# mmorise/World

Hardware: NVIDIA H100
Metric: analysis frames/sec (Harvest+CheapTrick+D4C) (higher is better)
Workload: dtype f64

## Files before the change

### world_b200/csrc/wb_f0common.cu

```cuda
#include "wb_internal.h"
#include "wb_f0common.cuh"
#include "wb_mma.cuh"
#include <stdlib.h>

namespace wb {

WB_KERNEL(256, 3) fir_plain_kernel(FirParams p) {
  WB_DYN_SMEM(double, smem);
  const int tid = WB_TID, nth = WB_NTH;
  const int T = 2048, R = 8, G = T / R;
  const int u = blockIdx.y, n0 = blockIdx.x * T;
  const int qlen = p.base_len[u] + p.extra_len;
  if (n0 >= qlen) return;
  const int ntaps = p.ntaps;
  const int seg_len = T + ntaps - 1;
  const int seg_cap = seg_len + 16;
  double *seg = smem;
  double *hrev = seg + (seg_cap + (seg_cap >> 3) + 8);
  const double *in = p.in + (size_t)u * p.in_stride + p.in_origin;
  double *out = p.out + (size_t)u * p.out_stride + p.out_origin;
  for (int j = tid; j < ntaps + 8; j += nth) hrev[j] = j < ntaps ? __ldg(&p.taps_rev[j]) : 0.0;
  const int m0 = n0 - ntaps + 1;
  for (int i = tid; i < seg_len + 8; i += nth) seg[pad8(i)] = (i < seg_len) ? in[m0 + i] : 0.0;
  WB_SYNC();
// ... 18 lines not shown
}

#ifndef WB_RING
#define WB_RING 256
#endif
#define WB_FCHUNK 256
struct Trains {
  const double *g[4];
  double *xr, *yr;
  int cap;
  int ifrom[4];
  double afs;
};
WB_DEV double edge_at(const Trains &T, int q, int i) {
  int s = i;
  while (s >= T.cap) s -= T.cap;
  return T.g[q][s];
}
WB_DEV double loc_at(const Trains &T, int q, int j) {
  return j >= T.ifrom[q] ? T.xr[q * WB_RING + (j & (WB_RING - 1))] : (edge_at(T, q, j) + edge_at(T, q, j + 1)) / 2.0 / T.afs;
}
WB_DEV double val_at(const Trains &T, int q, int j) {
  return j >= T.ifrom[q] ? T.yr[q * WB_RING + (j & (WB_RING - 1))] : T.afs / (edge_at(T, q, j + 1) - edge_at(T, q, j));
}

WB_DEV double train_value(const Trains &T, int q, int count, int n_int, double t) {
  const int k = imin(n_int - 1, imax(1, count));
  const double x0 = loc_at(T, q, k - 1), x1 = loc_at(T, q, k);
  const double y0 = val_at(T, q, k - 1), y1 = val_at(T, q, k);
  const double s = (t - x0) / (x1 - x0);
  return y0 + s * (y1 - y0);
}

WB_DEV int first_frame_at_or_after(double x, double frame_period) {
  int g = (int)ceil(x * 1000.0 / frame_period);
  if (g < 0) g = 0;
  while (g > 0 && !((g - 1) * frame_period / 1000.0 < x)) --g;
  while (g * frame_period / 1000.0 < x) ++g;
  return g;
}

#ifdef WB_EMU
static inline void smem_add_u64(unsigned long long *p, unsigned long long v) { *p += v; }
#else
__device__ __forceinline__ void smem_add_u64(unsigned long long *p, unsigned long long v) { atomicAdd(p, v); }
#endif

WB_DEV unsigned long long scan_packed(unsigned long long *c, int G, unsigned long long carry,
                                      unsigned long long *warp_tot ) {
#ifdef WB_EMU
  (void)warp_tot;
  unsigned long long run = carry;
  for (int g = 0; g < G; ++g) { const unsigned long long v = c[g]; c[g] = run; run += v; }
  return run;
#else
  const int tid = threadIdx.x, lane = tid & 31, w = tid >> 5, nw = G >> 5;
  const unsigned long long v = c[tid];
  unsigned long long inc = v;
  for (int o = 1; o < 32; o <<= 1) {
    const unsigned long long t = __shfl_up_sync(0xffffffffu, inc, o);
    if (lane >= o) inc += t;
  }
  if (lane == 31) warp_tot[w] = inc;
  __syncthreads();
  unsigned long long base = carry, all = carry;
  for (int i = 0; i < nw; ++i) { const unsigned long long t = warp_tot[i]; if (i < w) base += t; all += t; }
  c[tid] = base + inc - v;
  __syncthreads();
  return all;
#endif
}

WB_DEV void sweep_store_candidate(const SweepParams &p, int grp, double v0, double v1, double v2, double v3, int i,
                                  double bf, double *cand, double *score) {
  double c = (v0 + v1 + v2 + v3) / 4.0, sc = 0.0;
  const double f0_floor = grp < 0 ? p.f0_floor : p.grp_floor[grp], f0_ceil = grp < 0 ? p.f0_ceil : p.grp_ceil[grp];
  if (p.mode == 0) {
    sc = sqrt(((v0 - c) * (v0 - c) + (v1 - c) * (v1 - c) + (v2 - c) * (v2 - c) + (v3 - c) * (v3 - c)) / 3.0);
    if (c > bf || c < bf / 2.0 || c > f0_ceil || c < f0_floor) { c = 0.0; sc = 100000.0; }
  } else {
    if (c > bf * 1.1 || c < bf * 0.9 || c > f0_ceil || c < f0_floor) c = 0.0;
  }
  cand[i] = c;
  if (score) score[i] = sc / (c + kTiny);
}

WB_DEV void finalize_frames(const SweepParams &p, int grp, const Trains &T, int *lo_j, const int *ni, int f_begin, int f_end,
                            unsigned long long *marks, unsigned long long *orig, unsigned long long *scan_tmp,
                            double bf, double *cand, double *score) {
  const int tid = WB_TID, nth = WB_NTH;
  for (int c0 = f_begin; c0 < f_end; c0 += WB_FCHUNK) {
    const int c1 = imin(f_end, c0 + WB_FCHUNK);
    for (int i = tid; i < WB_FCHUNK; i += nth) marks[i] = 0ull;
    WB_SYNC();
    for (int q = 0; q < 4; ++q)
      for (int j = lo_j[q] + tid; j < ni[q]; j += nth) {
        int m = first_frame_at_or_after(loc_at(T, q, j), p.frame_period);
        if (m < c0) m = c0;
        if (m < c1) smem_add_u64(&marks[m - c0], 1ull << (16 * q));
      }
    WB_SYNC();
    for (int i = tid; i < WB_FCHUNK; i += nth) orig[i] = marks[i];
    WB_SYNC();
    const unsigned long long all = scan_packed(marks, WB_FCHUNK, 0ull, scan_tmp);
    for (int i = tid; i < c1 - c0; i += nth) {
      const unsigned long long inc = marks[i] + orig[i];
      const double t = (c0 + i) * p.frame_period / 1000.0;
      const double v0 = train_value(T, 0, lo_j[0] + (int)(inc & 0xffffull), ni[0], t);
      const double v1 = train_value(T, 1, lo_j[1] + (int)((inc >> 16) & 0xffffull), ni[1], t);
      const double v2 = train_value(T, 2, lo_j[2] + (int)((inc >> 32) & 0xffffull), ni[2], t);
      const double v3 = train_value(T, 3, lo_j[3] + (int)((inc >> 48) & 0xffffull), ni[3], t);
      sweep_store_candidate(p, grp, v0, v1, v2, v3, c0 + i, bf, cand, score);
    }
    lo_j[0] += (int)(all & 0xffffull); lo_j[1] += (int)((all >> 16) & 0xffffull);
// ... 553 lines not shown
      for (int w = 0; w < G / 32; ++w) {
        unsigned m[32], c[32], wsum = 0u;
        for (int l = 0; l < 32; ++l) {
          const int g = 32 * w + l;
          double v[WB_FE_R + 2];
          fe_load_group(st, g, v);
          m[l] = fe_mask_group(v, n0 - 2 + R * g, ylen, true);
          c[l] = fe_counts(m[l]);
          wsum += c[l];
        }
        unsigned ex = 0u;
        for (int l = 0; l < 32; ++l) { fe_stage(m[l], c[l], ex, wsum, R * (32 * w + l), evl); ex += c[l]; }
        const int s1 = fe_byte(wsum, 0), s2 = s1 + fe_byte(wsum, 1), s3 = s2 + fe_byte(wsum, 2);
        const int d[4] = {tot[s][0] + done[0], tot[s][1] + done[1] - s1, tot[s][2] + done[2] - s2, tot[s][3] + done[3] - s3};
        fe_emit_list(st, evl, 0, 1, wsum, d, n0, fb[s].edges, fb[s].cap);
        for (int q = 0; q < 4; ++q) done[q] += fe_byte(wsum, q);
      }
      for (int q = 0; q < 4; ++q) tot[s][q] += done[q];
      c0[s] = st[pad8(T - 2)]; c1[s] = st[pad8(T - 1)];
    }
  }
  for (int s = 0; s < nslot; ++s) {
    int *ec = p.ev_count + ((size_t)u * p.n_bands + fb[s].band) * 4;
    bool over = false;
    for (int q = 0; q < 4; ++q) { ec[q] = tot[s][q]; over = over || tot[s][q] > fb[s].cap; }
    if (over) {
      ec[0] = -1;
      p.redo_list[(*p.redo_count)++] = u * p.n_bands + fb[s].band;
    }
  }
#endif
}

#define WB_IP_F 256
#define WB_IP_W 256
struct IpTrain {
  const double *e; int n_int; double afs;
};
WB_DEV double ip_loc(const IpTrain &T, int j) { return (T.e[j] + T.e[j + 1]) / 2.0 / T.afs; }
WB_DEV double ip_val(const IpTrain &T, int j) { return T.afs / (T.e[j + 1] - T.e[j]); }

WB_DEV int first_frame_fast(double x, double frame_period, double frames_per_second) {
  const double r = x * frames_per_second;
  const double c = ceil(r);
  const double gap = c - r;
  if (gap > 1e-6 && gap < 1.0 - 1e-6 && r > 1.0 && r < 1e7) return (int)c;
  return first_frame_at_or_after(x, frame_period);
}

WB_KERNEL(256, 4) band_interp_kernel(SweepParams p) {
  WB_SHARED double xw[4][WB_IP_W + 4], yw[4][WB_IP_W + 4];
  WB_SHARED unsigned long long marks[WB_IP_F + 40];
  WB_SHARED unsigned long long orig[WB_IP_F];
  WB_SHARED int more_flag[2];
  const int tid = WB_TID, nth = WB_NTH;
  int u;
  const int b = sweep_block(p, &u);
  const UttBands ub = utt_bands(p, u);
  const int *ec = p.ev_count + ((size_t)u * p.n_bands + b) * 4;
  if (ec[0] < 0) return;
  const int nf = p.n_frames[u];
  double *cand = p.cand + ((size_t)u * p.n_bands + b) * p.frame_stride;
  double *score = p.score ? p.score + ((size_t)u * p.n_bands + b) * p.frame_stride : nullptr;
  const double bf = p.boundary[ub.band0 + b];
  const int cap = p.edge_cap[ub.band0 + b];
  const double *edges = p.edges + (size_t)u * p.edge_stride + (size_t)p.edge_off[ub.band0 + b];
  IpTrain tr[4];
  bool ok = true;
  for (int q = 0; q < 4; ++q) {
    tr[q].e = edges + (size_t)q * cap; tr[q].afs = p.afs;
    tr[q].n_int = ec[q] < 2 ? 0 : ec[q] - 1;
    if (tr[q].n_int - 2 <= 0) ok = false;
  }
  if (!ok) {
    for (int i = tid; i < nf; i += nth) {
      cand[i] = 0.0;
      if (score) score[i] = 100000.0 / (0.0 + kTiny);
    }
    return;
  }
  int w_band = (int)(bf * 1.1 * (WB_IP_F * p.frame_period / 1000.0) * 1.65) + 24;
  if (w_band > WB_IP_W) w_band = WB_IP_W;
  const double fps = 1000.0 / p.frame_period;
  int cursor[4] = {0, 0, 0, 0};
  for (int c0 = 0; c0 < nf; c0 += WB_IP_F) {
    const int c1 = imin(nf, c0 + WB_IP_F);
    for (int i = tid; i < WB_IP_F; i += nth) marks[i] = 0ull;
    for (int i = tid; i < 2; i += nth) more_flag[i] = 0;
    int at[4] = {cursor[0], cursor[1], cursor[2], cursor[3]};
    int wbase[4] = {0, 0, 0, 0}, wlen[4] = {0, 0, 0, 0};
    WB_SYNC();
    bool more = true;
    for (int itn = 0; more; ++itn) {
      for (int q = 0; q < 4; ++q) {
        wbase[q] = imax(0, at[q] - 2);
        wlen[q] = imin(tr[q].n_int - wbase[q], at[q] - wbase[q] + w_band);
      }
      const int off1 = wlen[0], off2 = off1 + wlen[1], off3 = off2 + wlen[2], total = off3 + wlen[3];
      for (int j = tid; j < total; j += nth) {
        const int q = (j >= off1 ? 1 : 0) + (j >= off2 ? 1 : 0) + (j >= off3 ? 1 : 0);
        const int k = j - (q == 0 ? 0 : q == 1 ? off1 : q == 2 ? off2 : off3);
        const int wb = q == 0 ? wbase[0] : q == 1 ? wbase[1] : q == 2 ? wbase[2] : wbase[3];
        const int aq = q == 0 ? at[0] : q == 1 ? at[1] : q == 2 ? at[2] : at[3];
        const int wl = q == 0 ? wlen[0] : q == 1 ? wlen[1] : q == 2 ? wlen[2] : wlen[3];
        const int ni = q == 0 ? tr[0].n_int : q == 1 ? tr[1].n_int : q == 2 ? tr[2].n_int : tr[3].n_int;
        IpTrain T;
        T.e = edges + (size_t)q * cap; T.n_int = ni; T.afs = p.afs;
        const double x = ip_loc(T, wb + k);
        xw[q][k] = x; yw[q][k] = ip_val(T, wb + k);
        if (k >= aq - wb) {
          const int m = first_frame_fast(x, p.frame_period, fps);
          if (m < c1) {
            smem_add_u64(&marks[imax(m, c0) - c0], 1ull << (16 * q));
            if (k == wl - 1 && wb + wl < ni) more_flag[itn & 1] = 1;
          }
        }
      }
      WB_SYNC();
      more = more_flag[itn & 1] != 0;
      if (tid == 0) more_flag[(itn & 1) ^ 1] = 0;
      for (int q = 0; q < 4; ++q) at[q] = wbase[q] + wlen[q];
      if (more) WB_SYNC();
    }
    for (int i = tid; i < WB_IP_F; i += nth) orig[i] = marks[i];
    WB_SYNC();
    const unsigned long long all = scan_packed(marks, WB_IP_F, 0ull, marks + WB_IP_F + 4);
    for (int i = c0 + tid; i < c1; i += nth) {
      const unsigned long long inc = marks[i - c0] + orig[i - c0];
      const double t = i * p.frame_period / 1000.0;
      double v[4];
#pragma unroll
      for (int q = 0; q < 4; ++q) {
        const int cnt = cursor[q] + (int)((inc >> (16 * q)) & 0xffffull);
        const int k = imin(tr[q].n_int - 1, imax(1, cnt));
        double x0, x1, y0, y1;
        const int w0 = k - 1 - wbase[q];
        if (w0 >= 0 && w0 + 1 < wlen[q]) {
          x0 = xw[q][w0]; x1 = xw[q][w0 + 1]; y0 = yw[q][w0]; y1 = yw[q][w0 + 1];
        } else {
          x0 = ip_loc(tr[q], k - 1); x1 = ip_loc(tr[q], k);
          y0 = ip_val(tr[q], k - 1); y1 = ip_val(tr[q], k);
        }
        const double s = (t - x0) / (x1 - x0);
        v[q] = y0 + s * (y1 - y0);
      }
      sweep_store_candidate(p, ub.grp, v[0], v[1], v[2], v[3], i, bf, cand, score);
    }
    cursor[0] += (int)(all & 0xffffull); cursor[1] += (int)((all >> 16) & 0xffffull);
    cursor[2] += (int)((all >> 32) & 0xffffull); cursor[3] += (int)((all >> 48) & 0xffffull);
    WB_SYNC();
  }
}

WB_DEV double dec_ext(const double *__restrict__ x, int n, int lag, int nx, int i) {
#define WB_XIN(k) x[imin(n - 1, imax(0, (k) - lag))]
  if (i < 9) return 2 * WB_XIN(0) - WB_XIN(9 - i);
  if (i < 9 + nx) return WB_XIN(i - 9);
  return 2 * WB_XIN(nx - 1) - WB_XIN(nx - 2 - (i - (9 + nx)));
#undef WB_XIN
}

template <int kPass>
WB_KERNEL_PLAIN decimate_pass_kernel(DecimateParams p) {
  const int u = blockIdx.y;
  const int n = p.x_len[u];
  const int nx = n + 2 * p.lag, nt = nx + 18;
  const long long g = (long long)blockIdx.x * blockDim.x + threadIdx.x;
  const long long begin = g * WB_DEC_BLOCK;
  if (begin >= nt) return;
  const int end = (int)(begin + WB_DEC_BLOCK < nt ? begin + WB_DEC_BLOCK : nt);
  const int start = (int)(begin - WB_DEC_WARM > 0 ? begin - WB_DEC_WARM : 0);
  const double *x = p.x + (size_t)u * p.x_stride;
  double *tmp = p.tmp + (size_t)u * p.tmp_stride;
  double a[3], b[2];
  decimate_coefficients(p.ratio, a, b);
  double w0 = 0.0, w1 = 0.0, w2 = 0.0;
  if (kPass == 0) {
    for (int i = start; i < end; ++i) {
      const double wt = dec_ext(x, n, p.lag, nx, i) + a[0] * w0 + a[1] * w1 + a[2] * w2;
      if (i >= begin) tmp[i] = b[0] * wt + b[1] * w0 + b[1] * w1 + b[0] * w2;
      w2 = w1; w1 = w0; w0 = wt;
    }
  } else {
    const int nout = (nx - 1) / p.ratio + 1;
// ... 27 lines not shown
  const size_t smem = fir_plain_smem_bytes(p.ntaps);
#ifndef WB_EMU
  cudaFuncSetAttribute(fir_plain_kernel, cudaFuncAttributeMaxDynamicSharedMemorySize, (int)smem);
#endif
  WB_LAUNCH_COOP(fir_plain_kernel, dim3(tiles, n_utts), 256, smem, ctx->stream, p);
}

void launch_nyquist_bins(Ctx *ctx, const NyquistParams &p, unsigned n_utts) {
  WB_LAUNCH_COOP(nyquist_bins_kernel, dim3(n_utts), 256, 0, ctx->stream, p);
}

static dim3 sweep_grid(const SweepParams &p, unsigned n_utts) {
  return p.ugrp ? dim3((unsigned)p.n_blk_band) : dim3((unsigned)p.n_bands, n_utts);
}

void launch_band_sweep(Ctx *ctx, const SweepParams &p_in, unsigned n_utts) {
  SweepParams p = p_in;
  p.debug_skip = 0;
  if (const char *e = getenv("WB_SWEEP_DEBUG")) p.debug_skip = atoi(e);
  const size_t smem = sweep_smem_bytes(p.max_taps);
  if (p.ripple) {
#ifndef WB_EMU
    cudaFuncSetAttribute(band_sweep_ripple_kernel, cudaFuncAttributeMaxDynamicSharedMemorySize, (int)smem);
#endif
    WB_LAUNCH_COOP(band_sweep_ripple_kernel, sweep_grid(p, n_utts), WB_SWEEP_THREADS, smem, ctx->stream, p);
  } else {
#ifndef WB_EMU
    cudaFuncSetAttribute(band_sweep_kernel, cudaFuncAttributeMaxDynamicSharedMemorySize, (int)smem);
#endif
    WB_LAUNCH_COOP(band_sweep_kernel, sweep_grid(p, n_utts), WB_SWEEP_THREADS, smem, ctx->stream, p);
  }
}

void launch_band_sweep_split(Ctx *ctx, const SweepParams &p_in, unsigned n_utts) {
  SweepParams p = p_in;
  p.debug_skip = 0;
  const size_t smem_fe = fe_smem_bytes(p.max_taps), smem_sw = sweep_smem_bytes(p.max_taps);
#ifndef WB_EMU
  cudaFuncSetAttribute(band_fir_events_kernel, cudaFuncAttributeMaxDynamicSharedMemorySize, (int)smem_fe);
  cudaFuncSetAttribute(band_sweep_list_kernel, cudaFuncAttributeMaxDynamicSharedMemorySize, (int)smem_sw);
#endif
  const dim3 pair_grid = p.ugrp ? dim3((unsigned)p.n_blk_pair) : dim3((unsigned)((p.n_bands + 1) / 2), n_utts);
  WB_LAUNCH_COOP(band_fir_events_kernel, pair_grid, WB_SWEEP_THREADS, smem_fe, ctx->stream, p);
  WB_LAUNCH_COOP(band_interp_kernel, sweep_grid(p, n_utts), 256, 0, ctx->stream, p);
  WB_LAUNCH_COOP(band_sweep_list_kernel, dim3((unsigned)(3 * ctx->sm_count)), WB_SWEEP_THREADS, smem_sw, ctx->stream, p);
}

}
```

### world_b200/csrc/wb_f0common.cuh

```cuda
#pragma once
#include "wb_platform.cuh"
#include "wb_block.cuh"

namespace wb {

struct Ctx;

#define WB_SWEEP_T 2048
#define WB_SWEEP_R 8
#define WB_SWEEP_THREADS 256

WB_DEV int pad8(int i) { return i + (i >> 3); }

WB_HD inline void decimate_coefficients(int r, double a[3], double b[2]) {
  switch (r) {
    case 11: a[0] = 2.450743295230728; a[1] = -2.06794904601978; a[2] = 0.59574774438332101;
      b[0] = 0.0026822508007163792; b[1] = 0.0080467524021491377; break;
    case 12: a[0] = 2.4981398605924205; a[1] = -2.1368928194784025; a[2] = 0.62187513816221485;
      b[0] = 0.0021097275904709001; b[1] = 0.0063291827714127002; break;
    case 10: a[0] = 2.3936475118069387; a[1] = -1.9873904075111861; a[2] = 0.5658879979027055;
      b[0] = 0.0034818622251927556; b[1] = 0.010445586675578267; break;
    case 9: a[0] = 2.3236003491759578; a[1] = -1.8921545617463598; a[2] = 0.53148928133729068;
      b[0] = 0.0046331164041389372; b[1] = 0.013899349212416812; break;
    case 8: a[0] = 2.2357462340187593; a[1] = -1.7780899984041358; a[2] = 0.49152555365968692;
// ... 29 lines not shown
struct SweepParams {
  const double *sig; size_t sig_stride; int sig_origin;
  const int *y_len;
  int n_bands;
  const double *taps_rev; const int *tap_off; const int *ntaps; const int *shift;
  const double *boundary;
  double afs;
  double *edges; size_t edge_stride;
  const int *edge_cap; const long long *edge_off;
  const int *n_frames; int frame_stride; double frame_period;
  int mode;
  const double *nyq; int ripple;
  double f0_floor, f0_ceil;
  double *cand; double *score;
  int max_taps;
  int *status;
  int debug_skip;
  int *ev_count;
  int *redo_list; int *redo_count;
  const int *ugrp = nullptr; const int *grp_band0 = nullptr, *grp_nb = nullptr;
  const double *grp_floor = nullptr, *grp_ceil = nullptr;
  const int *blk0_band = nullptr, *blk0_pair = nullptr; int n_blk_band = 0, n_blk_pair = 0, n_utts = 0;
};

struct UttBands { int band0, nb, grp; };
WB_DEV UttBands utt_bands(const SweepParams &p, int u) {
  UttBands r;
  if (!p.ugrp) { r.band0 = 0; r.nb = p.n_bands; r.grp = -1; return r; }
  r.grp = p.ugrp[u];
  r.band0 = p.grp_band0[r.grp]; r.nb = p.grp_nb[r.grp];
  return r;
}

WB_DEV int flat_block(const int *first, int n_utts, int blk, int *u) {
  int lo = 0, hi = n_utts - 1;
  while (lo < hi) {
    const int mid = (lo + hi + 1) >> 1;
    if (first[mid] <= blk) lo = mid; else hi = mid - 1;
  }
  *u = lo;
  return blk - first[lo];
}

#define WB_FE_R 8
#define WB_FE_TILE (WB_FE_R * 128)
#define WB_FE_EVMAX 16
WB_HD inline int fe_kpad(int ntaps) { return (ntaps + 8 + 7) / 8 * 8; }
WB_HD inline int fe_seg_doubles(int max_taps) { return WB_FE_TILE + fe_kpad(max_taps) + 16; }
WB_HD inline int fe_hrev_doubles(int max_taps) { return fe_kpad(max_taps) + 16; }
WB_HD inline int fe_st_doubles() { return WB_FE_TILE + (WB_FE_TILE >> 3) + 8; }
WB_HD inline size_t fe_smem_bytes(int max_taps) {
  return (size_t)(2 * fe_seg_doubles(max_taps) + 2 * fe_hrev_doubles(max_taps) + 2 * fe_st_doubles() + 8 + 2 + 6) * 8 +
         (size_t)2 * 128 * WB_FE_EVMAX * 2;
}

WB_HD inline size_t sweep_smem_bytes(int max_taps) {
  const int seg = WB_SWEEP_T + max_taps + 16;
  return (size_t)(seg + (seg >> 3) + 8) * 8 + (size_t)(max_taps + 8) * 8 + (size_t)(WB_SWEEP_T + 8 + ((WB_SWEEP_T + 8) >> 3) + 8) * 8 +
         (size_t)(WB_SWEEP_T / WB_SWEEP_R + 40) * 8 + 8 * 256 * 8 + 2 * 256 * 8;
}

#define WB_DEC_BLOCK 256
#define WB_DEC_WARM 512
struct DecimateParams {
  const double *x; const int *x_len; int x_stride;
  int ratio, lag;
  double *tmp; size_t tmp_stride;
  double *y; size_t y_stride; int y_origin;
  int first;
  int n_out_mode;
};

void launch_decimate(Ctx *ctx, const DecimateParams &p, int max_x_len, unsigned n_utts);
void launch_fir_plain(Ctx *ctx, const FirParams &p, unsigned tiles, unsigned n_utts);
void launch_band_sweep(Ctx *ctx, const SweepParams &p, unsigned n_utts);
void launch_band_sweep_split(Ctx *ctx, const SweepParams &p, unsigned n_utts);

struct NyquistParams {
  const double *sig; size_t stride; int origin;
  const int *y_len; int c;
  const int *nfft;
  double *nyq;
};
void launch_nyquist_bins(Ctx *ctx, const NyquistParams &p, unsigned n_utts);

}
```

### world_b200/csrc/wb_harvest.cu

```cuda
#include "wb_internal.h"
#include "wb_f0common.cuh"
#include "wb_spectral.cuh"
#include "wb_mma.cuh"
#include <stdlib.h>
#include <stdio.h>
#include <string.h>
#include <map>
#include <string>
#include <vector>

namespace wb {

static void plan_edge_caps(const std::vector<double> &boundary, double afs, int max_ylen, bool full,
                           std::vector<int> *cap, std::vector<long long> *off, size_t *stride) {
  const int nb = (int)boundary.size();
  cap->resize(nb); off->resize(nb);
  long long run = 0;
  long long floor_cap = 2048;
  if (const char *e = getenv("WB_EDGE_CAP_MIN")) floor_cap = atoll(e) > 0 ? atoll(e) : floor_cap;
  for (int i = 0; i < nb; ++i) {
    const long long hard = (long long)max_ylen / 2 + 2;
    long long soft = (long long)(2.5 * boundary[i] * max_ylen / afs) + 64;
    if (soft < floor_cap) soft = floor_cap;
    if (full) soft = hard;
// ... 38 lines not shown
struct HvDetectParams {
  const double *raw; int n_bands; int l1_stride; const int *l1;
  HvGroups gr;
  double *base; int *base_count; int *nc;
  int n_utts;
};

WB_KERNEL_PLAIN harvest_detect_kernel(HvDetectParams p) {
  const long long g = (long long)blockIdx.x * blockDim.x + threadIdx.x;
  if (g >= (long long)p.n_utts * p.l1_stride) return;
  const int u = (int)(g / p.l1_stride), i = (int)(g % p.l1_stride);
  if (i >= p.l1[u]) return;
  const double *raw = p.raw + (size_t)u * p.n_bands * p.l1_stride + i;
  const int nb = p.gr.grp_nb[p.gr.ugrp[u]];
  double *out = p.base + (size_t)g * WB_HV_BASE;
  int count = 0, prev = 0, st = 0;
  double sum = 0.0;
  for (int j = 1; j < nb; ++j) {
    const int v = (j == nb - 1) ? 0 : (raw[(size_t)j * p.l1_stride] > 0 ? 1 : 0);
    if (v - prev == 1) { st = j; sum = 0.0; }
    if (v) sum += raw[(size_t)j * p.l1_stride];
    if (v - prev == -1) {
      if (j - st >= 10 && count < WB_HV_BASE) out[count++] = sum / (j - st);
    }
    prev = v;
  }
  for (int c = count; c < WB_HV_BASE; ++c) out[c] = 0.0;
  p.base_count[g] = count;
#ifdef WB_EMU
  if (count > p.nc[u]) p.nc[u] = count;
#else
  if (count > 0) atomicMax(&p.nc[u], count);
#endif
}

struct HvRefineParams {
  const double *y; size_t y_stride; int y_origin; const int *y_len; double afs;
  const double *base; const int *nc; int l1_stride; const int *l1; int max_cand;
  HvGroups gr;
  double *cand; double *score;
  const double2 *tw;
  int nwin_max;
};

#ifdef WB_EMU
#define WB_LANE 0
#define WB_LANES 1
WB_DEV double warp_sum(double v) { return v; }
#else
#define WB_LANE ((int)(threadIdx.x & 31))
#define WB_LANES 32
WB_DEV double warp_sum(double v) {
  for (int o = 16; o; o >>= 1) v += __shfl_xor_sync(0xffffffffu, v, o);
  return v;
}
#endif

WB_DEV double2 hv_tw(const double2 *__restrict__ tw, int idx) {
  double2 w = __ldg(&tw[idx & (WB_TW_N / 2 - 1)]);
  if (idx & (WB_TW_N / 2)) { w.x = -w.x; w.y = -w.y; }
  return w;
}

WB_DEV void hv_refine_one(const double *__restrict__ y, int y_len, double afs, double t, double f,
                          double f0_floor, double f0_ceil, const double2 *__restrict__ tw, double *wbuf,
                          double *xbuf, double *dbuf, double *out_f0, double *out_score) {
// ... 860 lines not shown
    sp.taps_rev = (const double *)(blk + o_taps); sp.tap_off = (const int *)(blk + o_toff);
    sp.ntaps = (const int *)(blk + o_nt); sp.shift = (const int *)(blk + o_sh);
    sp.boundary = (const double *)(blk + o_bd); sp.afs = afs;
    sp.edges = (double *)(blk + o_edges); sp.edge_stride = edge_stride;
    sp.edge_cap = (const int *)(blk + o_ecap); sp.edge_off = (const long long *)(blk + o_eoff);
    sp.n_frames = l1; sp.frame_stride = l1_stride; sp.frame_period = 1.0;
    sp.mode = 1; sp.f0_floor = groups[0].f0_floor; sp.f0_ceil = groups[0].f0_ceil;
    if (n_groups > 1) {
      sp.ugrp = gr.ugrp; sp.grp_band0 = (const int *)(blk + o_gb0); sp.grp_nb = gr.grp_nb;
      sp.grp_floor = gr.grp_floor; sp.grp_ceil = gr.grp_ceil;
      sp.blk0_band = (const int *)(blk + o_bband); sp.blk0_pair = (const int *)(blk + o_bpair);
      sp.n_blk_band = bband[n]; sp.n_blk_pair = bpair[n]; sp.n_utts = n;
    }
    sp.nyq = nullptr; sp.ripple = 0;
    if (ratio == 1 && !getenv("WB_NO_RIPPLE")) {
      std::vector<int> nfft(n);
      for (int i = 0; i < n; ++i) {
        const int xl = b.x_len_host ? b.x_len_host[u0 + i] : b.x_stride;
        const int yl = static_cast<int>(ceil(static_cast<double>(xl) / ratio));
        const int sample = yl + 5 + 2 * static_cast<int>(2.0 * afs / groups[ugrp[u0 + i]].boundary[0]);
        nfft[i] = static_cast<int>(pow(2.0, static_cast<int>(log(static_cast<double>(sample)) / kLog2) + 1.0));
      }
      rc = dev_memcpy_h2d(ctx, blk + o_nfft, nfft.data(), (size_t)n * 4);
      if (rc) return rc;
      NyquistParams np_;
      np_.sig = y; np_.stride = y_stride; np_.origin = padl; np_.y_len = ylen; np_.c = 0;
      np_.nfft = (const int *)(blk + o_nfft); np_.nyq = (double *)(blk + o_nyq);
      launch_nyquist_bins(ctx, np_, (unsigned)n);
      sp.nyq = (const double *)(blk + o_nyq); sp.ripple = 1;
    }
    sp.cand = (double *)(blk + o_raw); sp.score = nullptr;
    sp.max_taps = max_taps; sp.status = ctx->status_dev;
    sp.ev_count = (int *)(blk + o_evc); sp.redo_list = (int *)(blk + o_redo); sp.redo_count = (int *)(blk + o_nredo);
    if (!sp.ripple && !getenv("WB_SWEEP_STREAMING") && fe_smem_bytes(max_taps) <= 200 * 1024) {
      rc = dev_memset(ctx, sp.redo_count, 0, 4);
      if (rc) return rc;
      launch_band_sweep_split(ctx, sp, (unsigned)n);
    } else {
      launch_band_sweep(ctx, sp, (unsigned)n);
    }

#ifdef WB_EMU
    if (const char *dump = getenv("WB_DUMP_RAW")) {
      FILE *f = fopen(dump, "wb");
      if (f) { fwrite(sp.cand, 8, (size_t)n * nb * l1_stride, f); fclose(f); }
    }
#endif
    const long long slots = (long long)n * l1_stride;
    HvDetectParams dp;
    dp.raw = sp.cand; dp.n_bands = nb; dp.l1_stride = l1_stride; dp.l1 = l1; dp.gr = gr;
    dp.base = (double *)(blk + o_base); dp.base_count = (int *)(blk + o_bcnt); dp.nc = nc; dp.n_utts = n;
    WB_LAUNCH_FLAT(harvest_detect_kernel, dim3((unsigned)((slots + 127) / 128)), 128, 0, ctx->stream, dp);

#ifdef WB_EMU
    if (const char *dump = getenv("WB_DUMP_BASE")) {
      FILE *f = fopen(dump, "wb");
      if (f) { fwrite(dp.base, 8, (size_t)n * l1_stride * WB_HV_BASE, f); fclose(f); }
    }
#endif
    HvRefineParams rp;
    rp.y = y; rp.y_stride = y_stride; rp.y_origin = padl; rp.y_len = ylen; rp.afs = afs;
    rp.base = dp.base; rp.nc = nc; rp.l1_stride = l1_stride; rp.l1 = l1; rp.max_cand = max_cand;
    rp.gr = gr;
    rp.cand = (double *)(blk + o_c1); rp.score = (double *)(blk + o_s1); rp.tw = ctx->twiddle; rp.nwin_max = nwin_max;
#ifdef WB_EMU
    const unsigned refine_blocks = (unsigned)l1_stride;
#else
    const unsigned refine_blocks = (unsigned)((l1_stride + WB_HV_WARPS - 1) / WB_HV_WARPS);
#endif
    const int frame_samples = static_cast<int>(afs / 1000.0);
    if (!getenv("WB_NO_REFINE_CHAIN") && frame_samples >= 1 && frame_samples * 1000.0 == afs) {
      rc = dev_memset(ctx, rp.cand, 0, (size_t)n * l1_stride * max_cand * 8);
      if (!rc) rc = dev_memset(ctx, rp.score, 0, (size_t)n * l1_stride * max_cand * 8);
      if (rc) return rc;
      HvWindowParams wp;
      wp.win = (double *)(blk + o_win); wp.afs = afs;
      WB_LAUNCH_FLAT(harvest_window_table_kernel, dim3((unsigned)(nwin_max / 2 + 1)), 128, 0, ctx->stream, wp);
      HvChainParams chp;
      chp.r = rp; chp.frame_samples = frame_samples; chp.win = wp.win;
      const size_t smem_chain = (size_t)WB_HV_WARPS * hv_chain_seg(nwin_max, frame_samples) * 8;
#ifndef WB_EMU
      cudaFuncSetAttribute(harvest_refine_chain_kernel, cudaFuncAttributeMaxDynamicSharedMemorySize, (int)smem_chain);
#endif
      WB_LAUNCH_COOP(harvest_refine_chain_kernel, dim3(refine_blocks, (unsigned)n), 32 * WB_HV_WARPS, smem_chain, ctx->stream, chp);
    } else {
// ... 35 lines not shown
```

Before: 2.746 million.

## Fuse Harvest band interpolation with candidate detection into one kernel

Adds a kernel that walks each band's zero-crossing event trains per frame, interpolates the four trains and finds runs of valid candidates directly. It keeps the per-frame run state in shared memory, so the full per-band candidate array is no longer written and read back. The separate interpolation launch and the flat detect launch are skipped by default, and an environment variable restores the old path. The trade-off is sequential per-thread train walking and a per-segment binary-search startup, which may lower parallelism compared with the old per-band kernel.

Measured after the change: 2.847 million (median of 6 runs). 1.04x the previous value.

```diff
diff --git a/world_b200/csrc/wb_f0common.cu b/world_b200/csrc/wb_f0common.cu
--- a/world_b200/csrc/wb_f0common.cu
+++ b/world_b200/csrc/wb_f0common.cu
@@ -74,14 +74,6 @@
   return y0 + s * (y1 - y0);
 }
 
-WB_DEV int first_frame_at_or_after(double x, double frame_period) {
-  int g = (int)ceil(x * 1000.0 / frame_period);
-  if (g < 0) g = 0;
-  while (g > 0 && !((g - 1) * frame_period / 1000.0 < x)) --g;
-  while (g * frame_period / 1000.0 < x) ++g;
-  return g;
-}
-
 #ifdef WB_EMU
 static inline void smem_add_u64(unsigned long long *p, unsigned long long v) { *p += v; }
 #else
@@ -115,13 +107,14 @@
 
 WB_DEV void sweep_store_candidate(const SweepParams &p, int grp, double v0, double v1, double v2, double v3, int i,
                                   double bf, double *cand, double *score) {
-  double c = (v0 + v1 + v2 + v3) / 4.0, sc = 0.0;
-  const double f0_floor = grp < 0 ? p.f0_floor : p.grp_floor[grp], f0_ceil = grp < 0 ? p.f0_ceil : p.grp_ceil[grp];
+  double c, sc = 0.0;
   if (p.mode == 0) {
+    c = (v0 + v1 + v2 + v3) / 4.0;
+    const double f0_floor = grp < 0 ? p.f0_floor : p.grp_floor[grp], f0_ceil = grp < 0 ? p.f0_ceil : p.grp_ceil[grp];
     sc = sqrt(((v0 - c) * (v0 - c) + (v1 - c) * (v1 - c) + (v2 - c) * (v2 - c) + (v3 - c) * (v3 - c)) / 3.0);
     if (c > bf || c < bf / 2.0 || c > f0_ceil || c < f0_floor) { c = 0.0; sc = 100000.0; }
   } else {
-    if (c > bf * 1.1 || c < bf * 0.9 || c > f0_ceil || c < f0_floor) c = 0.0;
+    c = harvest_band_candidate(p, grp, v0, v1, v2, v3, bf);
   }
   cand[i] = c;
   if (score) score[i] = sc / (c + kTiny);
@@ -743,19 +736,6 @@
 
 #define WB_IP_F 256
 #define WB_IP_W 256
-struct IpTrain {
-  const double *e; int n_int; double afs;
-};
-WB_DEV double ip_loc(const IpTrain &T, int j) { return (T.e[j] + T.e[j + 1]) / 2.0 / T.afs; }
-WB_DEV double ip_val(const IpTrain &T, int j) { return T.afs / (T.e[j + 1] - T.e[j]); }
-
-WB_DEV int first_frame_fast(double x, double frame_period, double frames_per_second) {
-  const double r = x * frames_per_second;
-  const double c = ceil(r);
-  const double gap = c - r;
-  if (gap > 1e-6 && gap < 1.0 - 1e-6 && r > 1.0 && r < 1e7) return (int)c;
-  return first_frame_at_or_after(x, frame_period);
-}
 
 WB_KERNEL(256, 4) band_interp_kernel(SweepParams p) {
   WB_SHARED double xw[4][WB_IP_W + 4], yw[4][WB_IP_W + 4];
@@ -952,7 +932,7 @@
   }
 }
 
-void launch_band_sweep_split(Ctx *ctx, const SweepParams &p_in, unsigned n_utts) {
+void launch_band_sweep_split(Ctx *ctx, const SweepParams &p_in, unsigned n_utts, bool interp) {
   SweepParams p = p_in;
   p.debug_skip = 0;
   const size_t smem_fe = fe_smem_bytes(p.max_taps), smem_sw = sweep_smem_bytes(p.max_taps);
@@ -962,7 +942,7 @@
 #endif
   const dim3 pair_grid = p.ugrp ? dim3((unsigned)p.n_blk_pair) : dim3((unsigned)((p.n_bands + 1) / 2), n_utts);
   WB_LAUNCH_COOP(band_fir_events_kernel, pair_grid, WB_SWEEP_THREADS, smem_fe, ctx->stream, p);
-  WB_LAUNCH_COOP(band_interp_kernel, sweep_grid(p, n_utts), 256, 0, ctx->stream, p);
+  if (interp) WB_LAUNCH_COOP(band_interp_kernel, sweep_grid(p, n_utts), 256, 0, ctx->stream, p);
   WB_LAUNCH_COOP(band_sweep_list_kernel, dim3((unsigned)(3 * ctx->sm_count)), WB_SWEEP_THREADS, smem_sw, ctx->stream, p);
 }
 
diff --git a/world_b200/csrc/wb_f0common.cuh b/world_b200/csrc/wb_f0common.cuh
--- a/world_b200/csrc/wb_f0common.cuh
+++ b/world_b200/csrc/wb_f0common.cuh
@@ -85,6 +85,34 @@
   return r;
 }
 
+WB_DEV double harvest_band_candidate(const SweepParams &p, int grp, double v0, double v1, double v2, double v3, double bf) {
+  const double c = (v0 + v1 + v2 + v3) / 4.0;
+  const double f0_floor = grp < 0 ? p.f0_floor : p.grp_floor[grp], f0_ceil = grp < 0 ? p.f0_ceil : p.grp_ceil[grp];
+  return (c > bf * 1.1 || c < bf * 0.9 || c > f0_ceil || c < f0_floor) ? 0.0 : c;
+}
+
+WB_DEV int first_frame_at_or_after(double x, double frame_period) {
+  int g = (int)ceil(x * 1000.0 / frame_period);
+  if (g < 0) g = 0;
+  while (g > 0 && !((g - 1) * frame_period / 1000.0 < x)) --g;
+  while (g * frame_period / 1000.0 < x) ++g;
+  return g;
+}
+
+WB_DEV int first_frame_fast(double x, double frame_period, double frames_per_second) {
+  const double r = x * frames_per_second;
+  const double c = ceil(r);
+  const double gap = c - r;
+  if (gap > 1e-6 && gap < 1.0 - 1e-6 && r > 1.0 && r < 1e7) return (int)c;
+  return first_frame_at_or_after(x, frame_period);
+}
+
+struct IpTrain {
+  const double *e; int n_int; double afs;
+};
+WB_DEV double ip_loc(const IpTrain &T, int j) { return (T.e[j] + T.e[j + 1]) / 2.0 / T.afs; }
+WB_DEV double ip_val(const IpTrain &T, int j) { return T.afs / (T.e[j + 1] - T.e[j]); }
+
 WB_DEV int flat_block(const int *first, int n_utts, int blk, int *u) {
   int lo = 0, hi = n_utts - 1;
   while (lo < hi) {
@@ -127,7 +155,7 @@
 void launch_decimate(Ctx *ctx, const DecimateParams &p, int max_x_len, unsigned n_utts);
 void launch_fir_plain(Ctx *ctx, const FirParams &p, unsigned tiles, unsigned n_utts);
 void launch_band_sweep(Ctx *ctx, const SweepParams &p, unsigned n_utts);
-void launch_band_sweep_split(Ctx *ctx, const SweepParams &p, unsigned n_utts);
+void launch_band_sweep_split(Ctx *ctx, const SweepParams &p, unsigned n_utts, bool interp);
 
 struct NyquistParams {
   const double *sig; size_t stride; int origin;
diff --git a/world_b200/csrc/wb_harvest.cu b/world_b200/csrc/wb_harvest.cu
--- a/world_b200/csrc/wb_harvest.cu
+++ b/world_b200/csrc/wb_harvest.cu
@@ -94,6 +94,207 @@
 #else
   if (count > 0) atomicMax(&p.nc[u], count);
 #endif
+}
+
+#define WB_HI_THREADS 256
+#define WB_HI_RUNS 16
+#define WB_HI_L 16
+#define WB_HI_BC (WB_HI_THREADS / WB_HI_RUNS)
+#define WB_HI_SEG 2048
+#define WB_HI_CSTR (WB_HI_RUNS * (WB_HI_L + 1))
+static_assert(WB_HI_RUNS * WB_HI_L == WB_HI_THREADS, "one frame of a tile per thread in the fold");
+WB_HD inline size_t hi_smem_bytes() { return (size_t)WB_HI_BC * WB_HI_CSTR * 8 + (size_t)WB_HI_SEG * (8 + 4); }
+
+struct InterpDetectParams {
+  SweepParams s;
+  double *base; int *base_count; int *nc;
+};
+
+struct HiTrain {
+  IpTrain T;
+  int c;
+  int mc;
+  double e1, e2;
+  double x0, x1, y0, y1;
+};
+struct HiItem {
+  HiTrain tr[4];
+  int mode;
+};
+
+WB_DEV void hi_step(HiTrain &w, int i, const SweepParams &p, double fps) {
+  if (w.mc > i) return;
+  ++w.c;
+  if (w.c >= w.T.n_int) { w.mc = 0x7fffffff; return; }
+  const double x = (w.e1 + w.e2) / 2.0 / p.afs, y = p.afs / (w.e2 - w.e1);
+  w.mc = first_frame_fast(x, p.frame_period, fps);
+  w.e1 = w.e2;
+  if (w.c + 2 <= w.T.n_int) w.e2 = w.T.e[w.c + 2];
+  if (w.c >= 2) { w.x0 = w.x1; w.y0 = w.y1; w.x1 = x; w.y1 = y; }
+}
+
+WB_DEV void hi_advance(HiItem &h, int i, const SweepParams &p, double fps) {
+  while (h.tr[0].mc <= i || h.tr[1].mc <= i || h.tr[2].mc <= i || h.tr[3].mc <= i) {
+#pragma unroll
+    for (int q = 0; q < 4; ++q) hi_step(h.tr[q], i, p, fps);
+  }
+}
+
+WB_DEV void hi_start(HiItem &h, const SweepParams &p, const UttBands &ub, int u, int b, int f0, double fps) {
+  const int *ec = p.ev_count + ((size_t)u * p.n_bands + b) * 4;
+  if (ec[0] < 0) { h.mode = 2; return; }
+  const int cap = p.edge_cap[ub.band0 + b];
+  const double *edges = p.edges + (size_t)u * p.edge_stride + (size_t)p.edge_off[ub.band0 + b];
+  h.mode = 0;
+  int lo[4], hi[4];
+#pragma unroll
+  for (int q = 0; q < 4; ++q) {
+    HiTrain &w = h.tr[q];
+    w.T.e = edges + (size_t)q * cap; w.T.afs = p.afs;
+    w.T.n_int = ec[q] < 2 ? 0 : ec[q] - 1;
+    if (w.T.n_int - 2 <= 0) h.mode = 1;
+    lo[q] = 0; hi[q] = w.T.n_int;
+  }
+  if (h.mode) return;
+  for (bool busy = f0 > 0; busy;) {
+    busy = false;
+#pragma unroll
+    for (int q = 0; q < 4; ++q)
+      if (lo[q] < hi[q]) {
+        const int mid = (lo[q] + hi[q]) >> 1;
+        if (first_frame_fast(ip_loc(h.tr[q].T, mid), p.frame_period, fps) < f0) lo[q] = mid + 1; else hi[q] = mid;
+        busy = true;
+      }
+  }
+#pragma unroll
+  for (int q = 0; q < 4; ++q) {
+    HiTrain &w = h.tr[q];
+    const int c = f0 > 0 ? lo[q] : 0, n = w.T.n_int, k = imin(n - 1, imax(1, c));
+    w.c = c;
+    w.mc = c < n ? first_frame_fast(ip_loc(w.T, c), p.frame_period, fps) : 0x7fffffff;
+    w.e1 = c + 1 <= n ? w.T.e[c + 1] : 0.0;
+    w.e2 = c + 2 <= n ? w.T.e[c + 2] : 0.0;
+    w.x0 = ip_loc(w.T, k - 1); w.y0 = ip_val(w.T, k - 1);
+    w.x1 = ip_loc(w.T, k); w.y1 = ip_val(w.T, k);
+  }
+}
+
+WB_KERNEL(WB_HI_THREADS, 2) harvest_interp_detect_kernel(InterpDetectParams ip) {
+  const SweepParams &p = ip.s;
+  WB_DYN_SMEM(double, smem);
+  double *cbuf = smem;
+  double *fsum = cbuf + WB_HI_BC * WB_HI_CSTR;
+  int *fst = reinterpret_cast<int *>(fsum + WB_HI_SEG);
+  const int tid = WB_TID, nth = WB_NTH;
+  const int u = blockIdx.y;
+  const int nf = p.n_frames[u];
+  const int nseg = (nf + WB_HI_SEG - 1) / WB_HI_SEG;
+  if ((int)blockIdx.x >= nseg) return;
+  const int seg = (nf + nseg - 1) / nseg;
+  const int s0 = (int)blockIdx.x * seg, len = imin(seg, nf - s0);
+  if (len <= 0) return;
+  const int rl = (len + WB_HI_THREADS - 1) / WB_HI_THREADS * WB_HI_L;
+  const int n_tiles = rl / WB_HI_L;
+  const UttBands ub = utt_bands(p, u);
+  const double fps = 1000.0 / p.frame_period;
+  for (int f = tid; f < len; f += nth) { fsum[f] = 0.0; fst[f] = 0; }
+#ifdef WB_EMU
+  static HiItem items[WB_HI_THREADS];
+#define WB_HI_ITEM(it) items[it]
+#else
+  HiItem item;
+#define WB_HI_ITEM(it) item
+#endif
+  for (int b0 = 1; b0 < ub.nb - 1; b0 += WB_HI_BC) {
+    const int nbc = imin(WB_HI_BC, ub.nb - 1 - b0);
+    for (int it = tid; it < WB_HI_THREADS; it += nth) {
+      HiItem &h = WB_HI_ITEM(it);
+      const int bl = it / WB_HI_RUNS, r = it % WB_HI_RUNS;
+      h.mode = 3;
+      if (bl < nbc && r * rl < len) hi_start(h, p, ub, u, b0 + bl, s0 + r * rl, fps);
+    }
+    for (int tile = 0; tile < n_tiles; ++tile) {
+      for (int it = tid; it < WB_HI_THREADS; it += nth) {
+        HiItem &h = WB_HI_ITEM(it);
+        if (h.mode == 3) continue;
+        const int bl = it / WB_HI_RUNS, r = it % WB_HI_RUNS, b = b0 + bl;
+        const int fo0 = r * rl + tile * WB_HI_L;
+        const int n_fr = imin(WB_HI_L, len - fo0);
+        double *cb = cbuf + bl * WB_HI_CSTR + r * (WB_HI_L + 1);
+        const double bf = p.boundary[ub.band0 + b];
+        for (int pp = 0; pp < n_fr; ++pp) {
+          const int i = s0 + fo0 + pp;
+          double c = 0.0;
+          if (h.mode == 0) {
+            hi_advance(h, i, p, fps);
+            const double t = i * p.frame_period / 1000.0;
+            double v[4];
+#pragma unroll
+            for (int q = 0; q < 4; ++q) {
+              const HiTrain &w = h.tr[q];
+              const double s = (t - w.x0) / (w.x1 - w.x0);
+              v[q] = w.y0 + s * (w.y1 - w.y0);
+            }
+            c = harvest_band_candidate(p, ub.grp, v[0], v[1], v[2], v[3], bf);
+          } else if (h.mode == 2) {
+            c = p.cand[((size_t)u * p.n_bands + b) * p.frame_stride + i];
+          }
+          cb[pp] = c;
+        }
+      }
+      WB_SYNC();
+      for (int sl = tid; sl < WB_HI_THREADS; sl += nth) {
+        const int r = sl / WB_HI_L, pp = sl % WB_HI_L;
+        const int fo = r * rl + tile * WB_HI_L + pp;
+        if (fo >= len) continue;
+        const int s = fst[fo];
+        int prev = s & 1, count = (s >> 1) & 63, st = s >> 7;
+        double sum = fsum[fo];
+        double *out = ip.base + ((size_t)u * p.frame_stride + s0 + fo) * WB_HV_BASE;
+        const double *cb = cbuf + r * (WB_HI_L + 1) + pp;
+        for (int bl = 0; bl < nbc; ++bl) {
+          const int j = b0 + bl;
+          const double raw = cb[bl * WB_HI_CSTR];
+          const int v = raw > 0 ? 1 : 0;
+          if (v - prev == 1) { st = j; sum = 0.0; }
+          if (v) sum += raw;
+          if (v - prev == -1) {
+            if (j - st >= 10 && count < WB_HV_BASE) out[count++] = sum / (j - st);
+          }
+          prev = v;
+        }
+        fst[fo] = st << 7 | count << 1 | prev;
+        fsum[fo] = sum;
+      }
+      WB_SYNC();
+    }
+  }
+#undef WB_HI_ITEM
+  WB_SYNC();
+  for (int fo = tid; fo < len; fo += nth) {
+    const int s = fst[fo];
+    int count = (s >> 1) & 63;
+    const int j = ub.nb - 1, st = s >> 7;
+    const size_t g = (size_t)u * p.frame_stride + s0 + fo;
+    double *out = ip.base + g * WB_HV_BASE;
+    if ((s & 1) && j - st >= 10 && count < WB_HV_BASE) { out[count] = fsum[fo] / (j - st); ++count; }
+    for (int c = count; c < WB_HV_BASE; ++c) out[c] = 0.0;
+    ip.base_count[g] = count;
+#ifdef WB_EMU
+    if (count > ip.nc[u]) ip.nc[u] = count;
+#else
+    if (count > 0) atomicMax(&ip.nc[u], count);
+#endif
+  }
+}
+
+static void launch_interp_detect(Ctx *ctx, const InterpDetectParams &p, unsigned n_utts) {
+  const size_t smem = hi_smem_bytes();
+#ifndef WB_EMU
+  cudaFuncSetAttribute(harvest_interp_detect_kernel, cudaFuncAttributeMaxDynamicSharedMemorySize, (int)smem);
+#endif
+  const unsigned nseg = (unsigned)((p.s.frame_stride + WB_HI_SEG - 1) / WB_HI_SEG);
+  WB_LAUNCH_COOP(harvest_interp_detect_kernel, dim3(nseg, n_utts), WB_HI_THREADS, smem, ctx->stream, p);
 }
 
 struct HvRefineParams {
@@ -1020,25 +1221,25 @@
     sp.cand = (double *)(blk + o_raw); sp.score = nullptr;
     sp.max_taps = max_taps; sp.status = ctx->status_dev;
     sp.ev_count = (int *)(blk + o_evc); sp.redo_list = (int *)(blk + o_redo); sp.redo_count = (int *)(blk + o_nredo);
-    if (!sp.ripple && !getenv("WB_SWEEP_STREAMING") && fe_smem_bytes(max_taps) <= 200 * 1024) {
-      rc = dev_memset(ctx, sp.redo_count, 0, 4);
-      if (rc) return rc;
-      launch_band_sweep_split(ctx, sp, (unsigned)n);
-    } else {
-      launch_band_sweep(ctx, sp, (unsigned)n);
-    }
-
-#ifdef WB_EMU
-    if (const char *dump = getenv("WB_DUMP_RAW")) {
-      FILE *f = fopen(dump, "wb");
-      if (f) { fwrite(sp.cand, 8, (size_t)n * nb * l1_stride, f); fclose(f); }
-    }
-#endif
     const long long slots = (long long)n * l1_stride;
     HvDetectParams dp;
     dp.raw = sp.cand; dp.n_bands = nb; dp.l1_stride = l1_stride; dp.l1 = l1; dp.gr = gr;
     dp.base = (double *)(blk + o_base); dp.base_count = (int *)(blk + o_bcnt); dp.nc = nc; dp.n_utts = n;
-    WB_LAUNCH_FLAT(harvest_detect_kernel, dim3((unsigned)((slots + 127) / 128)), 128, 0, ctx->stream, dp);
+    if (!sp.ripple && !getenv("WB_SWEEP_STREAMING") && fe_smem_bytes(max_taps) <= 200 * 1024) {
+      const bool fused = !getenv("WB_HV_UNFUSED_DETECT");
+      rc = dev_memset(ctx, sp.redo_count, 0, 4);
+      if (rc) return rc;
+      launch_band_sweep_split(ctx, sp, (unsigned)n, !fused);
+      if (fused) {
+        InterpDetectParams ip;
+        ip.s = sp; ip.base = dp.base; ip.base_count = dp.base_count; ip.nc = nc;
+        launch_interp_detect(ctx, ip, (unsigned)n);
+      }
+      if (!fused) WB_LAUNCH_FLAT(harvest_detect_kernel, dim3((unsigned)((slots + 127) / 128)), 128, 0, ctx->stream, dp);
+    } else {
+      launch_band_sweep(ctx, sp, (unsigned)n);
+      WB_LAUNCH_FLAT(harvest_detect_kernel, dim3((unsigned)((slots + 127) / 128)), 128, 0, ctx->stream, dp);
+    }
 
 #ifdef WB_EMU
     if (const char *dump = getenv("WB_DUMP_BASE")) {
```

## Rewrite band interpolation as warp-per-row with shuffle-based edge windows

Applied to the files above, without the earlier changes.

Replaces the block-per-band interpolation kernel, which used shared-memory windows, atomic frame marks, a packed prefix scan and many block barriers, with one warp per (utterance, band) row. Each warp slides a 32-wide window of edge intervals in registers and finds each frame's interval with a shuffle-based binary search, advancing the window as frames pass. This removes shared-memory atomics, scans and __syncthreads from a small, latency-bound kernel and packs eight rows per block. The per-lane loop can become divergent when edge density is high relative to frame rate. The change also adds a non-emulator raw-candidate dump path that is active only when an environment variable is set.

After: 3.218 million before, 3.281 million after, median of 6. 1.02x the previous value.

```diff
diff --git a/world_b200/csrc/wb_f0common.cu b/world_b200/csrc/wb_f0common.cu
--- a/world_b200/csrc/wb_f0common.cu
+++ b/world_b200/csrc/wb_f0common.cu
@@ -741,13 +741,13 @@
 #endif
 }
 
-#define WB_IP_F 256
-#define WB_IP_W 256
-struct IpTrain {
-  const double *e; int n_int; double afs;
-};
-WB_DEV double ip_loc(const IpTrain &T, int j) { return (T.e[j] + T.e[j + 1]) / 2.0 / T.afs; }
-WB_DEV double ip_val(const IpTrain &T, int j) { return T.afs / (T.e[j + 1] - T.e[j]); }
+#define WB_IP_ROWS 8
+WB_DEV double ip_loc(double e0, double e1, double afs) { return (e0 + e1) / 2.0 / afs; }
+WB_DEV double ip_val(double e0, double e1, double afs) { return afs / (e1 - e0); }
+WB_DEV double ip_lerp(double t, double x0, double x1, double y0, double y1) {
+  const double s = (t - x0) / (x1 - x0);
+  return y0 + s * (y1 - y0);
+}
 
 WB_DEV int first_frame_fast(double x, double frame_period, double frames_per_second) {
   const double r = x * frames_per_second;
@@ -757,108 +757,133 @@
   return first_frame_at_or_after(x, frame_period);
 }
 
-WB_KERNEL(256, 4) band_interp_kernel(SweepParams p) {
-  WB_SHARED double xw[4][WB_IP_W + 4], yw[4][WB_IP_W + 4];
-  WB_SHARED unsigned long long marks[WB_IP_F + 40];
-  WB_SHARED unsigned long long orig[WB_IP_F];
-  WB_SHARED int more_flag[2];
-  const int tid = WB_TID, nth = WB_NTH;
-  int u;
-  const int b = sweep_block(p, &u);
+struct IpRow {
+  const double *e[4];
+  int n_int[4];
+  double *cand, *score;
+  double bf;
+  int nf, grp;
+};
+WB_DEV bool ip_row(const SweepParams &p, int r, int lane, int nl, IpRow &R) {
+  int u, b;
+  if (!p.ugrp) { u = r / p.n_bands; b = r - u * p.n_bands; }
+  else b = flat_block(p.blk0_band, p.n_utts, r, &u);
   const UttBands ub = utt_bands(p, u);
   const int *ec = p.ev_count + ((size_t)u * p.n_bands + b) * 4;
-  if (ec[0] < 0) return;
-  const int nf = p.n_frames[u];
-  double *cand = p.cand + ((size_t)u * p.n_bands + b) * p.frame_stride;
-  double *score = p.score ? p.score + ((size_t)u * p.n_bands + b) * p.frame_stride : nullptr;
-  const double bf = p.boundary[ub.band0 + b];
+  if (ec[0] < 0) return false;
+  R.nf = p.n_frames[u]; R.grp = ub.grp; R.bf = p.boundary[ub.band0 + b];
+  R.cand = p.cand + ((size_t)u * p.n_bands + b) * p.frame_stride;
+  R.score = p.score ? p.score + ((size_t)u * p.n_bands + b) * p.frame_stride : nullptr;
   const int cap = p.edge_cap[ub.band0 + b];
   const double *edges = p.edges + (size_t)u * p.edge_stride + (size_t)p.edge_off[ub.band0 + b];
-  IpTrain tr[4];
   bool ok = true;
   for (int q = 0; q < 4; ++q) {
-    tr[q].e = edges + (size_t)q * cap; tr[q].afs = p.afs;
-    tr[q].n_int = ec[q] < 2 ? 0 : ec[q] - 1;
-    if (tr[q].n_int - 2 <= 0) ok = false;
-  }
-  if (!ok) {
-    for (int i = tid; i < nf; i += nth) {
-      cand[i] = 0.0;
-      if (score) score[i] = 100000.0 / (0.0 + kTiny);
-    }
-    return;
-  }
-  int w_band = (int)(bf * 1.1 * (WB_IP_F * p.frame_period / 1000.0) * 1.65) + 24;
-  if (w_band > WB_IP_W) w_band = WB_IP_W;
-  const double fps = 1000.0 / p.frame_period;
-  int cursor[4] = {0, 0, 0, 0};
-  for (int c0 = 0; c0 < nf; c0 += WB_IP_F) {
-    const int c1 = imin(nf, c0 + WB_IP_F);
-    for (int i = tid; i < WB_IP_F; i += nth) marks[i] = 0ull;
-    for (int i = tid; i < 2; i += nth) more_flag[i] = 0;
-    int at[4] = {cursor[0], cursor[1], cursor[2], cursor[3]};
-    int wbase[4] = {0, 0, 0, 0}, wlen[4] = {0, 0, 0, 0};
-    WB_SYNC();
-    bool more = true;
-    for (int itn = 0; more; ++itn) {
-      for (int q = 0; q < 4; ++q) {
-        wbase[q] = imax(0, at[q] - 2);
-        wlen[q] = imin(tr[q].n_int - wbase[q], at[q] - wbase[q] + w_band);
-      }
-      const int off1 = wlen[0], off2 = off1 + wlen[1], off3 = off2 + wlen[2], total = off3 + wlen[3];
-      for (int j = tid; j < total; j += nth) {
-        const int q = (j >= off1 ? 1 : 0) + (j >= off2 ? 1 : 0) + (j >= off3 ? 1 : 0);
-        const int k = j - (q == 0 ? 0 : q == 1 ? off1 : q == 2 ? off2 : off3);
-        const int wb = q == 0 ? wbase[0] : q == 1 ? wbase[1] : q == 2 ? wbase[2] : wbase[3];
-        const int aq = q == 0 ? at[0] : q == 1 ? at[1] : q == 2 ? at[2] : at[3];
-        const int wl = q == 0 ? wlen[0] : q == 1 ? wlen[1] : q == 2 ? wlen[2] : wlen[3];
-        const int ni = q == 0 ? tr[0].n_int : q == 1 ? tr[1].n_int : q == 2 ? tr[2].n_int : tr[3].n_int;
-        IpTrain T;
-        T.e = edges + (size_t)q * cap; T.n_int = ni; T.afs = p.afs;
-        const double x = ip_loc(T, wb + k);
-        xw[q][k] = x; yw[q][k] = ip_val(T, wb + k);
-        if (k >= aq - wb) {
-          const int m = first_frame_fast(x, p.frame_period, fps);
-          if (m < c1) {
-            smem_add_u64(&marks[imax(m, c0) - c0], 1ull << (16 * q));
-            if (k == wl - 1 && wb + wl < ni) more_flag[itn & 1] = 1;
-          }
-        }
-      }
-      WB_SYNC();
-      more = more_flag[itn & 1] != 0;
-      if (tid == 0) more_flag[(itn & 1) ^ 1] = 0;
-      for (int q = 0; q < 4; ++q) at[q] = wbase[q] + wlen[q];
-      if (more) WB_SYNC();
-    }
-    for (int i = tid; i < WB_IP_F; i += nth) orig[i] = marks[i];
-    WB_SYNC();
-    const unsigned long long all = scan_packed(marks, WB_IP_F, 0ull, marks + WB_IP_F + 4);
-    for (int i = c0 + tid; i < c1; i += nth) {
-      const unsigned long long inc = marks[i - c0] + orig[i - c0];
+    R.e[q] = edges + (size_t)q * cap;
+    R.n_int[q] = ec[q] < 2 ? 0 : ec[q] - 1;
+    if (R.n_int[q] - 2 <= 0) ok = false;
+  }
+  if (!ok)
+    for (int i = lane; i < R.nf; i += nl) {
+      R.cand[i] = 0.0;
+      if (R.score) R.score[i] = 100000.0 / (0.0 + kTiny);
+    }
+  return ok;
+}
+
+#ifndef WB_EMU
+#define WB_FULL 0xffffffffu
+struct IpWin {
+  int wb;
+  int m, m31;
+  double x, y;
+  double na, nb;
+};
+WB_DEV void ip_advance(IpWin &w, const double *e, int n_int, int lane, double afs, double frame_period, double fps) {
+  w.wb += 31;
+  const int j = w.wb + lane;
+  w.x = ip_loc(w.na, w.nb, afs);
+  w.y = ip_val(w.na, w.nb, afs);
+  w.m = j < n_int ? first_frame_fast(w.x, frame_period, fps) : 0x7fffffff;
+  w.m31 = __shfl_sync(WB_FULL, w.m, 31);
+  if (j + 31 < n_int) { w.na = __ldg(e + j + 31); w.nb = __ldg(e + j + 32); }
+}
+WB_DEV int ip_count(const IpWin &w, int i) {
+  int c = 0;
+#pragma unroll
+  for (int s = 16; s >= 1; s >>= 1)
+    if (__shfl_sync(WB_FULL, w.m, c + s - 1) <= i) c += s;
+  return (c == 31 && w.m31 <= i) ? 32 : c;
+}
+WB_DEV double ip_value(const IpWin &w, int n_int, int c, double t) {
+  const int k = imin(n_int - 1, imax(1, w.wb + c));
+  const int l0 = imin(30, imax(0, k - 1 - w.wb));
+  const double x0 = __shfl_sync(WB_FULL, w.x, l0), x1 = __shfl_sync(WB_FULL, w.x, l0 + 1);
+  const double y0 = __shfl_sync(WB_FULL, w.y, l0), y1 = __shfl_sync(WB_FULL, w.y, l0 + 1);
+  return ip_lerp(t, x0, x1, y0, y1);
+}
+#endif
+
+WB_KERNEL(32 * WB_IP_ROWS, 2) band_interp_kernel(SweepParams p, int n_rows) {
+  const double fps = 1000.0 / p.frame_period, afs = p.afs;
+#ifdef WB_EMU
+  for (int r = blockIdx.x * WB_IP_ROWS; r < imin(n_rows, (int)(blockIdx.x + 1) * WB_IP_ROWS); ++r) {
+    IpRow R;
+    if (!ip_row(p, r, 0, 1, R)) continue;
+    int cnt[4] = {0, 0, 0, 0};
+    for (int i = 0; i < R.nf; ++i) {
       const double t = i * p.frame_period / 1000.0;
       double v[4];
-#pragma unroll
       for (int q = 0; q < 4; ++q) {
-        const int cnt = cursor[q] + (int)((inc >> (16 * q)) & 0xffffull);
-        const int k = imin(tr[q].n_int - 1, imax(1, cnt));
-        double x0, x1, y0, y1;
-        const int w0 = k - 1 - wbase[q];
-        if (w0 >= 0 && w0 + 1 < wlen[q]) {
-          x0 = xw[q][w0]; x1 = xw[q][w0 + 1]; y0 = yw[q][w0]; y1 = yw[q][w0 + 1];
-        } else {
-          x0 = ip_loc(tr[q], k - 1); x1 = ip_loc(tr[q], k);
-          y0 = ip_val(tr[q], k - 1); y1 = ip_val(tr[q], k);
-        }
-        const double s = (t - x0) / (x1 - x0);
-        v[q] = y0 + s * (y1 - y0);
-      }
-      sweep_store_candidate(p, ub.grp, v[0], v[1], v[2], v[3], i, bf, cand, score);
-    }
-    cursor[0] += (int)(all & 0xffffull); cursor[1] += (int)((all >> 16) & 0xffffull);
-    cursor[2] += (int)((all >> 32) & 0xffffull); cursor[3] += (int)((all >> 48) & 0xffffull);
-    WB_SYNC();
-  }
+        const double *e = R.e[q];
+        while (cnt[q] < R.n_int[q] && first_frame_fast(ip_loc(e[cnt[q]], e[cnt[q] + 1], afs), p.frame_period, fps) <= i) ++cnt[q];
+        const int k = imin(R.n_int[q] - 1, imax(1, cnt[q]));
+        v[q] = ip_lerp(t, ip_loc(e[k - 1], e[k], afs), ip_loc(e[k], e[k + 1], afs), ip_val(e[k - 1], e[k], afs), ip_val(e[k], e[k + 1], afs));
+      }
+      sweep_store_candidate(p, R.grp, v[0], v[1], v[2], v[3], i, R.bf, R.cand, R.score);
+    }
+  }
+#else
+  const int lane = threadIdx.x & 31;
+  const int r = blockIdx.x * WB_IP_ROWS + (threadIdx.x >> 5);
+  IpRow R;
+  if (r >= n_rows || !ip_row(p, r, lane, 32, R)) return;
+  IpWin w[4];
+#pragma unroll
+  for (int q = 0; q < 4; ++q) {
+    w[q].wb = -31; w[q].na = 0.0; w[q].nb = 0.0;
+    if (lane < R.n_int[q]) { w[q].na = __ldg(R.e[q] + lane); w[q].nb = __ldg(R.e[q] + lane + 1); }
+  }
+#pragma unroll
+  for (int q = 0; q < 4; ++q) ip_advance(w[q], R.e[q], R.n_int[q], lane, afs, p.frame_period, fps);
+  for (int c0 = 0; c0 < R.nf; c0 += 32) {
+    const int i = c0 + lane;
+    const double t = i * p.frame_period / 1000.0;
+    int c[4];
+    double v[4];
+#pragma unroll
+    for (int q = 0; q < 4; ++q) c[q] = ip_count(w[q], i);
+#pragma unroll
+    for (int q = 0; q < 4; ++q) v[q] = ip_value(w[q], R.n_int[q], c[q], t);
+    bool later[4];
+#pragma unroll
+    for (int q = 0; q < 4; ++q) later[q] = i < R.nf && c[q] == 32 && w[q].wb + 32 < R.n_int[q];
+    while (__any_sync(WB_FULL, later[0] || later[1] || later[2] || later[3])) {
+#pragma unroll
+      for (int q = 0; q < 4; ++q)
+        if (__any_sync(WB_FULL, later[q])) ip_advance(w[q], R.e[q], R.n_int[q], lane, afs, p.frame_period, fps);
+#pragma unroll
+      for (int q = 0; q < 4; ++q) c[q] = ip_count(w[q], i);
+#pragma unroll
+      for (int q = 0; q < 4; ++q) {
+        const double vq = ip_value(w[q], R.n_int[q], c[q], t);
+        const bool still = later[q] && c[q] == 32 && w[q].wb + 32 < R.n_int[q];
+        if (later[q] && !still) v[q] = vq;
+        later[q] = still;
+      }
+    }
+    if (i < R.nf) sweep_store_candidate(p, R.grp, v[0], v[1], v[2], v[3], i, R.bf, R.cand, R.score);
+  }
+#endif
 }
 
 WB_DEV double dec_ext(const double *__restrict__ x, int n, int lag, int nx, int i) {
@@ -962,7 +987,8 @@
 #endif
   const dim3 pair_grid = p.ugrp ? dim3((unsigned)p.n_blk_pair) : dim3((unsigned)((p.n_bands + 1) / 2), n_utts);
   WB_LAUNCH_COOP(band_fir_events_kernel, pair_grid, WB_SWEEP_THREADS, smem_fe, ctx->stream, p);
-  WB_LAUNCH_COOP(band_interp_kernel, sweep_grid(p, n_utts), 256, 0, ctx->stream, p);
+  const int n_rows = p.ugrp ? p.n_blk_band : p.n_bands * (int)n_utts;
+  WB_LAUNCH_COOP(band_interp_kernel, dim3((unsigned)((n_rows + WB_IP_ROWS - 1) / WB_IP_ROWS)), 32 * WB_IP_ROWS, 0, ctx->stream, p, n_rows);
   WB_LAUNCH_COOP(band_sweep_list_kernel, dim3((unsigned)(3 * ctx->sm_count)), WB_SWEEP_THREADS, smem_sw, ctx->stream, p);
 }
 
diff --git a/world_b200/csrc/wb_harvest.cu b/world_b200/csrc/wb_harvest.cu
--- a/world_b200/csrc/wb_harvest.cu
+++ b/world_b200/csrc/wb_harvest.cu
@@ -1020,6 +1020,11 @@
     sp.cand = (double *)(blk + o_raw); sp.score = nullptr;
     sp.max_taps = max_taps; sp.status = ctx->status_dev;
     sp.ev_count = (int *)(blk + o_evc); sp.redo_list = (int *)(blk + o_redo); sp.redo_count = (int *)(blk + o_nredo);
+    const char *dump_raw = getenv("WB_DUMP_RAW");
+    if (dump_raw) {
+      rc = dev_memset(ctx, sp.cand, 0, (size_t)n * nb * l1_stride * 8);
+      if (rc) return rc;
+    }
     if (!sp.ripple && !getenv("WB_SWEEP_STREAMING") && fe_smem_bytes(max_taps) <= 200 * 1024) {
       rc = dev_memset(ctx, sp.redo_count, 0, 4);
       if (rc) return rc;
@@ -1028,12 +1033,14 @@
       launch_band_sweep(ctx, sp, (unsigned)n);
     }
 
-#ifdef WB_EMU
-    if (const char *dump = getenv("WB_DUMP_RAW")) {
-      FILE *f = fopen(dump, "wb");
-      if (f) { fwrite(sp.cand, 8, (size_t)n * nb * l1_stride, f); fclose(f); }
-    }
-#endif
+    if (dump_raw) {
+      std::vector<double> raw((size_t)n * nb * l1_stride);
+      rc = dev_memcpy_d2h(ctx, raw.data(), sp.cand, raw.size() * 8);
+      if (!rc) rc = dev_sync(ctx);
+      if (rc) return rc;
+      FILE *f = fopen(dump_raw, "wb");
+      if (f) { fwrite(raw.data(), 8, raw.size(), f); fclose(f); }
+    }
     const long long slots = (long long)n * l1_stride;
     HvDetectParams dp;
     dp.raw = sp.cand; dp.n_bands = nb; dp.l1_stride = l1_stride; dp.l1 = l1; dp.gr = gr;
```
